# yizhiwang96/Slice3D

Measured on AMD Instinct MI355X. Metric: occupancy query-points/sec (U-Net encode + per-query decode, 256^2 x 12 slices), higher is better.
Workload: dtype f16x3

## Files before the change

### include/slice3d_hip.h

```cpp
#ifndef SLICE3D_HIP_H
#define SLICE3D_HIP_H

#include <stddef.h>
#include <stdint.h>

#ifdef __cplusplus
extern "C" {
#endif

#define S3D_VERSION 119
#define S3D_E_ARG (-1)
#define S3D_E_WORKSPACE (-2)

#define S3D_N_LEVELS 5
#define S3D_D_MODEL 128
#define S3D_N_LAYERS 3
#define S3D_FFN 2048
#define S3D_N_TOKENS_MAX 13

#define S3D_PREC_F32 0
#define S3D_PREC_F16X3 1
#define S3D_PREC_F16 2
#define S3D_PREC_BF16 3

int s3d_version(void);
// ... 325 lines not shown
```

### slice3d_amd/csrc/api.hip

```cpp
#include <dlfcn.h>
#include <stdarg.h>
#include <string.h>

#include <vector>
#include <mutex>

#include <math.h>

#include "conv.h"
#include "decode.h"
#include "train.h"
#include "ldm_ops.h"

static thread_local char g_err[512] = "";

void s3d_set_error(const char* fmt, ...) {
    va_list ap;
    va_start(ap, fmt);
    vsnprintf(g_err, sizeof(g_err), fmt, ap);
    va_end(ap);
}

extern "C" int s3d_version(void) { return S3D_VERSION; }
extern "C" const char* s3d_last_error(void) { return g_err; }
// ... 100 lines not shown
static const bool kEncTap[13] = {false, true, false, true, false, false, true,
                                 false, false, true, false, false, true};
static const int kUpC[4] = {512, 256, 128, 64};

struct PackedConv {
    size_t w, scale, shift;
    size_t w16;
    int cout_pad, KU;
};
struct EncLayout {
    PackedConv enc[13];
    size_t pool_scale[4], pool_shift[4];
};
struct UNetLayout {
    EncLayout E;
    PackedConv trans_c, trans_up[4], up_t[4], up_c1[4], up_c2[4], outc;
    size_t emds;
    size_t enc0_raw;
    size_t total;
};

static int pad16(int c) { return (c + 15) / 16 * 16; }

struct ImageAlloc {
    size_t off = 0;
    size_t take(size_t n) {
        size_t o = off;
        off += (n + 3) / 4 * 4;
        return o;
    }
    void conv(PackedConv& pc, int cout_pad, int KU) {
        pc.cout_pad = cout_pad;
        pc.KU = KU;
        pc.w = take((size_t)cout_pad * KU * 16);
        pc.w16 = take((size_t)cout_pad * KU * 16);
        pc.scale = take(cout_pad);
        pc.shift = take(cout_pad);
    }
};

static EncLayout enc_layout(ImageAlloc& a) {
    EncLayout E;
    for (int i = 0; i < 13; ++i) a.conv(E.enc[i], kEncCout[i], 9 * pad16(kEncCin[i]) / 16);
    const int tapc[4] = {64, 128, 256, 512};
    for (int i = 0; i < 4; ++i) {
        E.pool_scale[i] = a.take(tapc[i]);
        E.pool_shift[i] = a.take(tapc[i]);
    }
    return E;
}

static UNetLayout unet_layout(int n_slices) {
    UNetLayout L;
    ImageAlloc a;
    L.E = enc_layout(a);
    a.conv(L.trans_c, 512, 640 / 16);
    for (int i = 0; i < 4; ++i) {
        const int C = kUpC[i], Ct = C / 2;
        a.conv(L.trans_up[i], Ct, C / 16);
        a.conv(L.up_t[i], 4 * Ct, C / 16);
        a.conv(L.up_c1[i], Ct, 2 * 9 * Ct / 16);
        a.conv(L.up_c2[i], Ct, 9 * Ct / 16);
    }
    a.conv(L.outc, 16, 32 / 16);
    L.emds = a.take((size_t)n_slices * 128);
    L.enc0_raw = a.take(64 * 27);
    L.total = a.off;
    return L;
}

extern "C" size_t s3d_unet_packed_bytes(int n_slices) { return unet_layout(n_slices).total * sizeof(float); }

static int pack_conv3(const float* w, float* dst, int cout, int cout_pad, int cin_tot, int cin_begin, int cseg,
                      int KU_total, int u_off, int taps, hipStream_t st, int f16 = 0) {
    PackArgs a = {};
    a.f16 = f16;
// ... 22 lines not shown
        TRY(pack_conv3(P[i].w, base + pc.w, kEncCout[i], pc.cout_pad, kEncCin[i], 0, kEncCin[i], pc.KU, 0, 9, st));
        if (kEncCin[i] % 32 == 0)
            TRY(pack_conv3(P[i].w, base + pc.w16, kEncCout[i], pc.cout_pad, kEncCin[i], 0, kEncCin[i], pc.KU, 0, 9, st, 1));
        if (kEncTap[i])
            TRY(launch_fold_bn(P[i].b, nullptr, base + pc.scale, base + pc.shift, kEncCout[i], pc.cout_pad, 1, 0, st));
        else
            TRY(launch_fold_bn(P[i].b, P[i].bn, base + pc.scale, base + pc.shift, kEncCout[i], pc.cout_pad, 1, 1, st));
    }
    const int tapi[4] = {1, 3, 6, 9};
    for (int i = 0; i < 4; ++i)
        TRY(launch_fold_bn(nullptr, P[tapi[i]].bn, base + E.pool_scale[i], base + E.pool_shift[i], kEncCout[tapi[i]],
                           kEncCout[tapi[i]], 1, 0, st));
    return 0;
}

extern "C" int s3d_unet_pack(const S3dUNetParams* P, void* packed, size_t packed_bytes, void* stream) {
    hipStream_t st = (hipStream_t)stream;
    S3D_CHECK_ARG(P && packed, "unet_pack: null argument");
    S3D_CHECK_ARG(P->n_slices >= 1 && P->n_slices <= 12, "unet_pack: n_slices %d", P->n_slices);
    const UNetLayout L = unet_layout(P->n_slices);
    if (packed_bytes < L.total * sizeof(float)) {
        s3d_set_error("unet_pack: packed buffer %zu < %zu bytes", packed_bytes, L.total * sizeof(float));
        return S3D_E_WORKSPACE;
    }
    float* base = (float*)packed;
    TRY(pack_encoder(P->enc, base, L.E, st));
    if (hipMemcpyAsync(base + L.enc0_raw, P->enc[0].w, 64 * 27 * sizeof(float), hipMemcpyDeviceToDevice, st) != hipSuccess) {
        s3d_set_error("unet_pack: copy of conv1_1's weight failed");
        return S3D_E_ARG;
    }
    TRY(pack_linear(P->trans_c.w, base + L.trans_c.w, 512, 512, 640, 640, 0, st));
    TRY(pack_linear(P->trans_c.w, base + L.trans_c.w16, 512, 512, 640, 640, 0, st, 1));
    TRY(launch_fold_bn(P->trans_c.b, nullptr, base + L.trans_c.scale, base + L.trans_c.shift, 512, 512, 1, 0, st));
    for (int i = 0; i < 4; ++i) {
        const int C = kUpC[i], Ct = C / 2;
        TRY(pack_linear(P->trans_up[i].w, base + L.trans_up[i].w, Ct, Ct, C, C, 0, st));
        TRY(pack_linear(P->trans_up[i].w, base + L.trans_up[i].w16, Ct, Ct, C, C, 0, st, 1));
        TRY(launch_fold_bn(P->trans_up[i].b, nullptr, base + L.trans_up[i].scale, base + L.trans_up[i].shift, Ct,
                           Ct, 1, 0, st));
        {
            PackArgs a = {};
            a.src = P->up_t[i].w; a.dst = base + L.up_t[i].w; a.kind = S3D_PACK_CONVT;
            a.n_valid = 4 * Ct; a.n_pad = 4 * Ct; a.KU_total = C / 16; a.u_off = 0; a.ku_seg = C / 16;
            a.k_valid = C; a.ct = Ct;
            TRY(launch_pack(a, st));
            a.f16 = 1; a.dst = base + L.up_t[i].w16;
            TRY(launch_pack(a, st));
            TRY(launch_fold_bn(P->up_t[i].b, nullptr, base + L.up_t[i].scale, base + L.up_t[i].shift, Ct, 4 * Ct, 4,
                               0, st));
        }
        TRY(pack_conv3(P->up_c1[i].w, base + L.up_c1[i].w, Ct, Ct, C, 0, Ct, L.up_c1[i].KU, 0, 9, st));
        TRY(pack_conv3(P->up_c1[i].w, base + L.up_c1[i].w, Ct, Ct, C, Ct, Ct, L.up_c1[i].KU, 9 * Ct / 16, 9, st));
        TRY(pack_conv3(P->up_c1[i].w, base + L.up_c1[i].w16, Ct, Ct, C, 0, Ct, L.up_c1[i].KU, 0, 9, st, 1));
        TRY(pack_conv3(P->up_c1[i].w, base + L.up_c1[i].w16, Ct, Ct, C, Ct, Ct, L.up_c1[i].KU, 9 * Ct / 16, 9, st, 1));
        TRY(launch_fold_bn(nullptr, P->up_c1[i].bn, base + L.up_c1[i].scale, base + L.up_c1[i].shift, Ct, Ct, 1, 0,
                           st));
        TRY(pack_conv3(P->up_c2[i].w, base + L.up_c2[i].w, Ct, Ct, Ct, 0, Ct, L.up_c2[i].KU, 0, 9, st));
        TRY(pack_conv3(P->up_c2[i].w, base + L.up_c2[i].w16, Ct, Ct, Ct, 0, Ct, L.up_c2[i].KU, 0, 9, st, 1));
        TRY(launch_fold_bn(nullptr, P->up_c2[i].bn, base + L.up_c2[i].scale, base + L.up_c2[i].shift, Ct, Ct, 1, 0,
                           st));
    }
    TRY(pack_linear(P->outc.w, base + L.outc.w, 3, 16, 32, 32, 0, st));
    TRY(pack_linear(P->outc.w, base + L.outc.w16, 3, 16, 32, 32, 0, st, 1));
    TRY(launch_fold_bn(P->outc.b, nullptr, base + L.outc.scale, base + L.outc.shift, 3, 16, 1, 0, st));
    hipError_t e = hipMemcpyAsync(base + L.emds, P->emds, (size_t)P->n_slices * 128 * sizeof(float),
                                  hipMemcpyDeviceToDevice, st);
    if (e != hipSuccess) {
        s3d_set_error("unet_pack: memcpy failed: %s", hipGetErrorString(e));
        return (int)e;
    }
    return 0;
}

#define S3D_SPLITK_FLOATS ((size_t)4718592)
struct UNetWs {
    size_t in16, a, b, x[5], p[4], proj, up, mid, splitk;
    size_t total;
};
static UNetWs unet_ws(int B, int S, int ns) {
    UNetWs W;
    size_t off = 0;
    auto take = [&](size_t n) {
        size_t o = off;
        off += (n + 63) / 64 * 64;
        return o;
    };
    const size_t px = (size_t)B * S * S;
    W.in16 = take(px * 16);
    W.a = take(px * 64);
    W.b = take(px * 64 / 2);
    const int xc[5] = {64, 128, 256, 512, 512};
    for (int i = 0; i < 5; ++i) W.x[i] = take((px >> (2 * i)) * xc[i]);
    for (int i = 0; i < 4; ++i) W.p[i] = take((px >> (2 * (i + 1))) * xc[i]);
    W.proj = take(px * 32);
    W.up = take(px * ns * 32);
    W.mid = take(px * ns * 32);
    W.splitk = take(S3D_SPLITK_FLOATS);
    W.total = off;
    return W;
}

extern "C" size_t s3d_unet_workspace_bytes(int batch, int size, int n_slices) {
    return unet_ws(batch, size, n_slices).total * sizeof(float);
}

static ConvLaunch conv_desc(const float* base, const PackedConv& pc, int prec, int N, int H, int W, int ks, int act) {
    ConvLaunch c = {};
    c.wpk16 = prec != S3D_PREC_F32 ? (const void*)(base + pc.w16) : nullptr;
    c.single_pass = prec == S3D_PREC_F16;
    c.N = N; c.H = H; c.W = W; c.ks = ks;
    c.CoutPad = pc.cout_pad; c.wpk = base + pc.w; c.KU = pc.KU;
    c.scale = base + pc.scale; c.shift = base + pc.shift;
// ... 2 lines not shown
}
static ConvSrc plain_src(const float* p, int C) { return ConvSrc{p, C, 1, 0, 0}; }

static ConvLaunch proj_desc(const float* w, const void* w16, bool single, int n, int k, const float* x, int N, int H,
                            int W, float* out, const float* shift = nullptr, int act = S3D_ACT_NONE) {
    ConvLaunch c = {};
    c.N = N; c.H = H; c.W = W; c.ks = 1;
    c.CoutPad = n; c.wpk = w; c.KU = k / 16;
    c.wpk16 = w16; c.single_pass = single;
    c.shift = shift; c.act = act;
    c.out_mode = S3D_OUT_NHWC; c.cout_store = n; c.out_cstride = n;
    c.nsrc = 1;
    c.src[0] = plain_src(x, k);
    c.out = out;
    return c;
}

static int encoder_fwd(const float* base, const EncLayout& E, int prec, int N, int S, int first, const float* in,
                       float* const tap[5], float* const pp[2], float* const pool[4], float* splitk, hipStream_t st) {
    const float* cur = in;
    int curC = first ? kEncCout[0] : 16, res = S, tap_i = 0, flip = first;
    for (int i = first; i < 13; ++i) {
        ConvLaunch c = conv_desc(base, E.enc[i], prec, N, res, res, 3, kEncTap[i] ? S3D_ACT_NONE : S3D_ACT_RELU);
        c.nsrc = 1;
        c.src[0] = plain_src(cur, curC);
        c.splitk_ws = splitk; c.splitk_floats = S3D_SPLITK_FLOATS;
        c.out = kEncTap[i] ? tap[tap_i] : pp[flip];
        TRY(launch_conv(c, st));
        cur = c.out;
        curC = kEncCout[i];
// ... 29 lines not shown
        s3d_set_error("unet_encode: workspace %zu < %zu bytes", workspace_bytes, W.total * sizeof(float));
        return S3D_E_WORKSPACE;
    }
    const float* base = (const float*)packed;
    float* ws = (float*)workspace;

    ProfScope prof_(S3D_PROF_UNET, st);
    float* const pp[2] = {ws + W.a, ws + W.b};
    float* const tap[5] = {ws + W.x[0], ws + W.x[1], ws + W.x[2], ws + W.x[3], ws + W.x[4]};
    float* const pool[4] = {ws + W.p[0], ws + W.p[1], ws + W.p[2], ws + W.p[3]};
    TRY(launch_conv3x3_first(img, 3, base + L.enc0_raw, nullptr, pp[0], B, S, S, st, base + L.E.enc[0].scale,
                             base + L.E.enc[0].shift, 1));
    TRY(encoder_fwd(base, L.E, prec, B, S, 1, pp[0], tap, pp, pool, ws + W.splitk, st));
    const int r5 = S / 16;
    {
        ConvLaunch c = conv_desc(base, L.trans_c, prec, B * ns, r5, r5, 1, S3D_ACT_NONE);
        c.nsrc = 2;
        c.src[0] = ConvSrc{ws + W.x[4], 512, ns, 0, 0};
        c.src[1] = ConvSrc{base + L.emds, 128, 1, ns, 1};
        c.out = out->level[0];
        TRY(launch_conv(c, st));
    }
    const float* prev = out->level[0];
    int rp = r5;
    for (int i = 0; i < 4; ++i) {
        const int C = kUpC[i], Ct = C / 2, ro = rp * 2;
        {
            ConvLaunch c = conv_desc(base, L.trans_up[i], prec, B, ro, ro, 1, S3D_ACT_NONE);
            c.nsrc = 1;
            c.src[0] = plain_src(ws + W.x[3 - i], C);
            c.out = ws + W.proj;
            TRY(launch_conv(c, st));
        }
        {
            ConvLaunch c = conv_desc(base, L.up_t[i], prec, B * ns, rp, rp, 1, S3D_ACT_NONE);
            c.nsrc = 1;
            c.src[0] = plain_src(prev, C);
            c.out = ws + W.up;
            c.out_mode = S3D_OUT_CONVT;
            c.cout_store = Ct;
            TRY(launch_conv(c, st));
        }
        {
            ConvLaunch c = conv_desc(base, L.up_c1[i], prec, B * ns, ro, ro, 3, S3D_ACT_RELU);
            c.nsrc = 2;
            c.src[0] = ConvSrc{ws + W.proj, Ct, ns, 0, 0};
            c.src[1] = plain_src(ws + W.up, Ct);
            c.out = ws + W.mid;
            TRY(launch_conv(c, st));
        }
        {
            ConvLaunch c = conv_desc(base, L.up_c2[i], prec, B * ns, ro, ro, 3, S3D_ACT_RELU);
            c.nsrc = 1;
            c.src[0] = plain_src(ws + W.mid, Ct);
            c.out = out->level[i + 1];
            TRY(launch_conv(c, st));
        }
        prev = out->level[i + 1];
        rp = ro;
    }
    if (slices_rec) {
        ConvLaunch c = conv_desc(base, L.outc, prec, B * ns, S, S, 1, S3D_ACT_TANH);
        c.nsrc = 1;
        c.src[0] = plain_src(prev, 32);
// ... 687 lines not shown
```

### slice3d_amd/csrc/conv.h

```cpp
#pragma once
#include "common.h"
#include "dropout.h"

struct ConvSrc {
    const float* p;
    int C;
    int bdiv, bmod, sbcast;
};

#define S3D_GN_SLICES 64
#define S3D_GN_CMAX 1536
struct ConvGn {
    const float* table;
    int silu;
};

enum { S3D_ACT_NONE = 0, S3D_ACT_RELU = 1, S3D_ACT_TANH = 2 };
enum { S3D_OUT_NHWC = 0, S3D_OUT_CONVT = 1, S3D_OUT_NCHW = 2 };

struct ConvLaunch {
    ConvSrc src[2];
    int nsrc;
    int N, H, W;
    int ks;
// ... 10 lines not shown
    int act;
    float* out;
    int out_mode;
    int cout_store;
    int out_cstride;
    const float* residual;
    int out_accumulate;
    int xcd_remap;
    const float* gate;
    float gate_scale;
    unsigned long long drop_base;
    float* splitk_ws;
    size_t splitk_floats;
    DropCfg drop;
    ConvGn gn;
    int* splits_out;
};

int launch_conv(const ConvLaunch& a, hipStream_t stream);
int launch_conv_splitk_finish(const ConvLaunch& a, int nsplit, hipStream_t stream);

enum { S3D_PACK_LINEAR = 0, S3D_PACK_CONV = 1, S3D_PACK_CONVT = 2, S3D_PACK_CONV_DGRAD = 3,
       S3D_PACK_CONVT_DGRAD = 4, S3D_PACK_LINEAR_T = 5 };
struct PackArgs {
    const float* src;
    float* dst;
    int kind;
    int n_valid, n_pad;
    int KU_total, u_off, ku_seg;
    int ld, k_valid;
// ... 16 lines not shown
};
class PackBatchSuspend {
public:
    PackBatchSuspend();
    ~PackBatchSuspend();
private:
    void* saved_;
};
int launch_fold_bn(const float* bias, const float* const bn[4], float* scale, float* shift, int c_valid,
                   int c_pad, int rep, int bias_before_bn, hipStream_t stream);

int launch_bn_relu_pool(const float* in, const float* scale, const float* shift, float* out, int n, int h,
                        int w, int c, hipStream_t stream);
int launch_nchw_to_nhwc(const float* in, float* out, int n, int c, int h, int w, int cpad, hipStream_t stream);
int launch_nhwc_to_nchw(const float* in, float* out, int n, int c, int h, int w, hipStream_t stream);
int launch_add_nchw(const float* a, const float* b, float* out, int n, int c, int h, int w, hipStream_t stream);

int launch_vgg_prep(const float* pred, const float* target, const float* mean, const float* stdv, float* out,
                    int n_img, int size, hipStream_t stream);
int launch_vgg_first_f16x3(const float* pred, const float* target, const float* mean, const float* stdv, const float* w_oihw,
                           const float* bias, float* out, int n_img, int size, hipStream_t stream);
int launch_l1_diff(const float* a, const float* b, long n, float scale, float* partial, float* loss_acc,
                   hipStream_t stream);
```

### slice3d_amd/csrc/conv.hip

```cpp
#include <stdlib.h>
#include "conv.h"
#include <vector>

template <int MT, int NT>
__device__ __forceinline__ void conv_epilogue(const ConvLaunch& a, f32x4 (&acc)[MT][NT], const int (&pn)[MT],
                                              const int (&py)[MT], const int (&px)[MT], const bool (&pv)[MT],
                                              int jt0, int g) {
    const bool convt32 = a.out_mode == S3D_OUT_CONVT && a.cout_store % 32 == 0;
    if (NT % 2 == 0 && (a.out_mode == S3D_OUT_NHWC || convt32)) {
        const int m = threadIdx.x & 15;
        const bool lo = m < 8;
#pragma unroll
        for (int np = 0; np < NT / 2; ++np) {
            const int co = (jt0 + 2 * np) * 16 + 16 * (m >> 3) + 4 * g;
            const f32x4 sc = a.scale ? ld4(a.scale + co) : f32x4{1.f, 1.f, 1.f, 1.f};
            const f32x4 sh = a.shift ? ld4(a.shift + co) : zero4();
            const int ct = a.cout_store, cq = convt32 ? co / ct : 0, ccol = convt32 ? co - cq * ct : co;
            const bool col_ok = convt32 ? cq < 4 : co < a.cout_store;
#pragma unroll
            for (int mt = 0; mt < MT; ++mt) {
                f32x4 val[2];
                s3d_full_line_pair(acc[mt][2 * np], acc[mt][2 * np + 1], m, val[0], val[1]);
                const long ob = convt32 ? ((long)(pn[mt] * 2 * a.H + 2 * py[mt] + (cq >> 1)) * (2 * a.W) + 2 * px[mt] + (cq & 1)) * ct
                                        : ((long)(pn[mt] * a.H + py[mt]) * a.W + px[mt]) * a.out_cstride;
// ... 67 lines not shown
                const int ct = a.cout_store;
                const int q = co / ct, c = co - q * ct;
                if (q < 4) {
                    const int oy = 2 * py[mt] + (q >> 1), ox = 2 * px[mt] + (q & 1);
                    float* o = a.out + ((long)(pn[mt] * 2 * a.H + oy) * (2 * a.W) + ox) * ct + c;
                    st4(o, v);
                }
            } else {
#pragma unroll
                for (int i = 0; i < 4; ++i)
                    if (co + i < a.cout_store)
                        a.out[((long)(pn[mt] * a.cout_store + co + i) * a.H + py[mt]) * a.W + px[mt]] = v[i];
            }
        }
    }
}

__device__ __forceinline__ void conv_block_tile(const ConvLaunch& a, int n_co_blk, int& blk_co, long& blk_px) {
    const long L = blockIdx.x;
    if (!a.xcd_remap || n_co_blk == 1) {
        blk_co = (int)(L % n_co_blk);
        blk_px = L / n_co_blk;
        return;
    }
    const long n_px = gridDim.x / n_co_blk, full = n_px & ~7L, lim = full * n_co_blk;
    if (L < lim) {
        const long k = L >> 3;
        blk_co = (int)(k % n_co_blk);
        blk_px = (k / n_co_blk) * 8 + (L & 7);
    } else {
        const long r = L - lim;
        blk_co = (int)(r % n_co_blk);
        blk_px = full + r / n_co_blk;
    }
}

template <int MT, int NT, int WM, int WN, int KS>
__global__ __launch_bounds__(WM* WN * 64) void conv_igemm_kernel(const ConvLaunch a) {
    const int lane = threadIdx.x & 63;
    const int wave = threadIdx.x >> 6;
    const int wm = wave % WM, wn = wave / WM;
    const int m = lane & 15, g = lane >> 4;
    constexpr int PIX_WG = WM * MT * 16;
    constexpr int CO_WG = WN * NT * 16;
    const long P = (long)a.N * a.H * a.W;
    const int n_co_blk = a.CoutPad / CO_WG;
    int blk_co;
    long blk_px;
    conv_block_tile(a, n_co_blk, blk_co, blk_px);
    const int HW = a.H * a.W;
    const int stride = a.stride > 1 ? a.stride : 1;
    const int Hin = a.Hin ? a.Hin : a.H, Win = a.Win ? a.Win : a.W;
    const int PAD = a.pad_origin ? 0 : (KS == 3 ? 1 : 0);

    int pn[MT], py[MT], px[MT];
    bool pv[MT];
#pragma unroll
    for (int mt = 0; mt < MT; ++mt) {
        const long p = blk_px * PIX_WG + (long)(wm * MT + mt) * 16 + m;
        pv[mt] = p < P;
        const long pc = pv[mt] ? p : 0;
        pn[mt] = (int)(pc / HW);
        const int r = (int)(pc - (long)pn[mt] * HW);
        py[mt] = r / a.W;
        px[mt] = r - py[mt] * a.W;
    }

    f32x4 acc[MT][NT];
#pragma unroll
    for (int mt = 0; mt < MT; ++mt)
#pragma unroll
        for (int nt = 0; nt < NT; ++nt) acc[mt][nt] = zero4();

    const int jt0 = blk_co * (CO_WG / 16) + wn * NT;
    int ubase = 0;
#pragma unroll 1
    for (int s = 0; s < a.nsrc; ++s) {
        const ConvSrc S = a.src[s];
        const int cu = S.C >> 4;
#pragma unroll 1
        for (int tap = 0; tap < KS * KS; ++tap) {
            const int dy = tap / KS - PAD, dx = tap % KS - PAD;
            const float* bp[MT];
            bool ok[MT];
#pragma unroll
            for (int mt = 0; mt < MT; ++mt) {
                const int y = py[mt] * stride + dy, x = px[mt] * stride + dx;
                ok[mt] = pv[mt] && y >= 0 && y < Hin && x >= 0 && x < Win;
                const int ni = (S.bmod ? pn[mt] % S.bmod : pn[mt]) / S.bdiv;
// ... 8 lines not shown
                for (int mt = 0; mt < MT; ++mt) b[mt] = ok[mt] ? ld4(bp[mt] + 16 * c) : zero4();
#pragma unroll
                for (int nt = 0; nt < NT; ++nt) w[nt] = ld4(wp + ((size_t)nt * a.KU + c) * 256);
#pragma unroll
                for (int mt = 0; mt < MT; ++mt)
#pragma unroll
                    for (int nt = 0; nt < NT; ++nt) acc[mt][nt] += mfma4(w[nt], b[mt], zero4());
            }
        }
        ubase += KS * KS * cu;
    }

    conv_epilogue<MT, NT>(a, acc, pn, py, px, pv, jt0, g);
}

template <int MT, int NT, int WM, int WN, int KS>
__global__ __launch_bounds__(WM* WN * 64) void conv_igemm_f16x3_kernel(const ConvLaunch a) {
    const int lane = threadIdx.x & 63;
    const int wave = threadIdx.x >> 6;
    const int wm = wave % WM, wn = wave / WM;
    const int m = lane & 15, g = lane >> 4;
    constexpr int PIX_WG = WM * MT * 16;
    constexpr int CO_WG = WN * NT * 16;
    const long P = (long)a.N * a.H * a.W;
    const int n_co_blk = a.CoutPad / CO_WG;
    int blk_co;
    long blk_px;
    conv_block_tile(a, n_co_blk, blk_co, blk_px);
    const int HW = a.H * a.W;
    const int stride = a.stride > 1 ? a.stride : 1;
    const int Hin = a.Hin ? a.Hin : a.H, Win = a.Win ? a.Win : a.W;
// ... 1 lines not shown
    const int KU32 = a.KU >> 1;
    const _Float16* wimg = reinterpret_cast<const _Float16*>(a.wpk16);

    int pn[MT], py[MT], px[MT];
    bool pv[MT];
#pragma unroll
    for (int mt = 0; mt < MT; ++mt) {
        const long p = blk_px * PIX_WG + (long)(wm * MT + mt) * 16 + m;
        pv[mt] = p < P;
        const long pc = pv[mt] ? p : 0;
        pn[mt] = (int)(pc / HW);
        const int r = (int)(pc - (long)pn[mt] * HW);
        py[mt] = r / a.W;
        px[mt] = r - py[mt] * a.W;
    }
    f32x4 acc[MT][NT];
#pragma unroll
    for (int mt = 0; mt < MT; ++mt)
#pragma unroll
        for (int nt = 0; nt < NT; ++nt) acc[mt][nt] = zero4();

    const int jt0 = blk_co * (CO_WG / 16) + wn * NT;
    int ubase = 0;
#pragma unroll 1
    for (int s = 0; s < a.nsrc; ++s) {
        const ConvSrc S = a.src[s];
        const int cu = S.C >> 5;
#pragma unroll 1
        for (int tap = 0; tap < KS * KS; ++tap) {
            const int dy = tap / KS - PAD, dx = tap % KS - PAD;
            const float* bp[MT];
            bool ok[MT];
#pragma unroll
            for (int mt = 0; mt < MT; ++mt) {
                const int y = py[mt] * stride + dy, x = px[mt] * stride + dx;
                ok[mt] = pv[mt] && y >= 0 && y < Hin && x >= 0 && x < Win;
                const int ni = (S.bmod ? pn[mt] % S.bmod : pn[mt]) / S.bdiv;
// ... 413 lines not shown
__device__ unsigned long long c3_stamps[4][8];
#define C3_STAMP(i)                                                                                              \
    do {                                                                                                         \
        const long long t__ = wall_clock64();                                                                    \
        if (threadIdx.x == 0) atomicAdd(&c3_stamps[c3_cls][i], (unsigned long long)(t__ - c3_last));              \
        c3_last = t__;                                                                                           \
    } while (0)
extern "C" void s3d_debug_c3_stamps(unsigned long long* out) {
    unsigned long long z[32] = {0};
    (void)hipMemcpyFromSymbol(out, HIP_SYMBOL(c3_stamps), sizeof(z));
    (void)hipMemcpyToSymbol(HIP_SYMBOL(c3_stamps), z, sizeof(z));
}
#else
#define C3_STAMP(i)
#endif
template <int MT, int WP, int WC, int NBUF, bool GN = false>
__global__ __launch_bounds__(256) void conv3x3_lds_f16x3_kernel(const ConvLaunch a, int tiles_x, int tiles_y,
                                                                int chunks_per_split) {
    static_assert(MT * WP == 8 && WP * WC == 4, "tile is 8 rows, 4 waves");
    constexpr int NT = 2, CO_WG = WC * NT * 16;
    __shared__ __attribute__((aligned(16))) _Float16 s_in[NBUF][2][C3_HALO * C3_PXS];
    __shared__ __attribute__((aligned(16))) float s_gn[GN ? 2 * S3D_GN_CMAX : 4];
#ifdef C3_STAMPS
    long long c3_last = wall_clock64();
    const int c3_cls = gridDim.x == 96 ? 0 : gridDim.x == 48 ? 1 : gridDim.x == 12 ? 2 : 3;
    if (threadIdx.x == 0) atomicAdd(&c3_stamps[c3_cls][7], 1ull);
#endif
    const int lane = threadIdx.x & 63, wave = threadIdx.x >> 6;
    const int m = lane & 15, g = lane >> 4;
    const int wp = wave % WP, wc = wave / WP;
    const int n_co_blk = a.CoutPad / CO_WG;
    int blk_co;
// ... 70 lines not shown
    const int ch_lo = blockIdx.y * chunks_per_split;
    const int nchunk = min(cu0 + cu1, ch_lo + chunks_per_split);
    fetch(a.src[ch_lo < cu0 ? 0 : 1], ch_lo < cu0 ? ch_lo : ch_lo - cu0, ch_lo < cu0 ? 0 : a.src[0].C);
    if (GN) {
        const int Ct = a.src[0].C + (a.nsrc > 1 ? a.src[1].C : 0);
        const float* tb = a.gn.table + (size_t)n * 2 * Ct;
        for (int i = threadIdx.x; i < Ct / 4; i += 256) {
            st4(s_gn + 4 * i, ld4(tb + 4 * i));
            st4(s_gn + S3D_GN_CMAX + 4 * i, ld4(tb + Ct + 4 * i));
        }
        __syncthreads();
    }
    C3_STAMP(0);
    park(ch_lo & (NBUF - 1));
    C3_STAMP(1);
    __syncthreads();
    C3_STAMP(2);
#pragma unroll 1
    for (int ch = ch_lo; ch < nchunk; ++ch) {
        const int s = ch < cu0 ? 0 : 1, c = s ? ch - cu0 : ch, cu = s ? cu1 : cu0;
        const int ubase = s ? 9 * cu0 : 0;
        const _Float16* wp0 = wimg + ((size_t)jt0 * KU32 + ubase + c) * 1024 + lane * 8;
        s3d_half8 wh[NT], wl[NT];
#pragma unroll
        for (int nt = 0; nt < NT; ++nt) {
            const _Float16* f = wp0 + (size_t)nt * KU32 * 1024;
            wh[nt] = *reinterpret_cast<const s3d_half8*>(f);
            wl[nt] = *reinterpret_cast<const s3d_half8*>(f + 512);
        }
        if (ch + 1 < nchunk) {
// ... 364 lines not shown
            return 0;
        }
        return launch_conv_splitk_finish(a, splits, stream);
    }
    dim3 grid((unsigned)nblk, (unsigned)splits);
    constexpr int one_buf_max = 2;
    const bool one = cps <= one_buf_max;
    if (a.gn.table) {
        int ct = 0;
        for (int s = 0; s < a.nsrc; ++s) ct += a.src[s].C;
        S3D_CHECK_ARG(ct <= S3D_GN_CMAX, "conv: fused GroupNorm over %d channels", ct);
        if (co_wg == 64)
            hipLaunchKernelGGL((conv3x3_lds_f16x3_kernel<4, 2, 2, 2, true>), grid, dim3(256), 0, stream, a, tiles_x, tiles_y, cps);
        else
            hipLaunchKernelGGL((conv3x3_lds_f16x3_kernel<2, 4, 1, 2, true>), grid, dim3(256), 0, stream, a, tiles_x, tiles_y, cps);
    } else if (co_wg == 64) {
        hipLaunchKernelGGL((conv3x3_lds_f16x3_kernel<4, 2, 2, 2>), grid, dim3(256), 0, stream, a, tiles_x, tiles_y, cps);
    } else {
        if (one) hipLaunchKernelGGL((conv3x3_lds_f16x3_kernel<2, 4, 1, 1>), grid, dim3(256), 0, stream, a, tiles_x, tiles_y, cps);
        else hipLaunchKernelGGL((conv3x3_lds_f16x3_kernel<2, 4, 1, 2>), grid, dim3(256), 0, stream, a, tiles_x, tiles_y, cps);
    }
    S3D_LAUNCH_CHECK();
    if (a.splits_out) {
        *a.splits_out = splits;
        if (splits > 1) return 0;
    }
    if (splits > 1) return launch_conv_splitk_finish(a, splits, stream);
    return 0;
}

template <int MT, int NT, int WM, int WN>
static int launch_cfg(const ConvLaunch& a, hipStream_t stream) {
    constexpr int PIX_WG = WM * MT * 16, CO_WG = WN * NT * 16;
    const long P = (long)a.N * a.H * a.W;
    const long nblk = ((P + PIX_WG - 1) / PIX_WG) * (a.CoutPad / CO_WG);
    S3D_CHECK_ARG(nblk > 0 && nblk < (1L << 31), "conv grid out of range (%ld)", nblk);
    dim3 grid((unsigned)nblk), block(WM * WN * 64);
    bool f16 = a.wpk16 != nullptr && (a.KU % 2 == 0);
    for (int s = 0; s < a.nsrc; ++s) f16 = f16 && (a.src[s].C % 32 == 0);
    if (f16) {
        if (a.ks == 3)
            hipLaunchKernelGGL((conv_igemm_f16x3_kernel<MT, NT, WM, WN, 3>), grid, block, 0, stream, a);
        else if (a.ks == 2)
            hipLaunchKernelGGL((conv_igemm_f16x3_kernel<MT, NT, WM, WN, 2>), grid, block, 0, stream, a);
        else
            hipLaunchKernelGGL((conv_igemm_f16x3_kernel<MT, NT, WM, WN, 1>), grid, block, 0, stream, a);
        S3D_LAUNCH_CHECK();
        return 0;
    }
    if (a.ks == 3)
        hipLaunchKernelGGL((conv_igemm_kernel<MT, NT, WM, WN, 3>), grid, block, 0, stream, a);
    else if (a.ks == 2)
        hipLaunchKernelGGL((conv_igemm_kernel<MT, NT, WM, WN, 2>), grid, block, 0, stream, a);
    else
// ... 1 lines not shown
    S3D_LAUNCH_CHECK();
    return 0;
}

int launch_conv(const ConvLaunch& a_in, hipStream_t stream) {
    ConvLaunch a = a_in;
    a.xcd_remap = 1;
    S3D_CHECK_ARG(a.ks >= 1 && a.ks <= 3, "conv: ks must be 1, 2 or 3");
    S3D_CHECK_ARG(!a.pad_origin || (a.ks == 3 && a.stride > 1 && a.out_mode == S3D_OUT_NHWC),
                  "conv: pad_origin is served for strided 3x3 convolutions only");
    S3D_CHECK_ARG(a.CoutPad % 16 == 0 && a.CoutPad > 0, "conv: CoutPad %d", a.CoutPad);
    for (int s = 0; s < a.nsrc; ++s)
        S3D_CHECK_ARG(a.src[s].C % 16 == 0 && a.src[s].bdiv >= 1, "conv: bad source %d", s);
    S3D_CHECK_ARG(a.out_mode != S3D_OUT_CONVT || (a.drop.p <= 0.f && !a.gate && !a.residual && !a.out_accumulate),
                  "conv: ConvTranspose output takes no dropout / gate / residual / accumulate");
    if (conv3x3_lds_eligible(a)) return launch_conv3x3_lds(a, stream);
    S3D_CHECK_ARG(!a.gn.table, "conv: a fused GroupNorm needs the LDS-staged 3x3 kernel (ks 3, stride 1, channel counts multiples of 32)");
    if (conv1x1_small_eligible(a)) {
        bool served = false;
        const int rc = launch_conv1x1_small(a, stream, served);
        if (rc || served) return rc;
    }
    if (lin_stream_eligible(a)) return launch_lin_stream(a, stream);
    if (lin_rows_eligible(a)) return launch_lin_rows(a, stream);
    const long P = (long)a.N * a.H * a.W;
    const long want = 512;
    auto nblk = [&](int pix, int co) { return ((P + pix - 1) / pix) * (a.CoutPad / co); };
    if (a.CoutPad % 128 == 0) {
        if (nblk(128, 128) >= want) return launch_cfg<4, 4, 2, 2>(a, stream);
        if (nblk(64, 128) >= want) return launch_cfg<2, 4, 2, 2>(a, stream);
// ... 218 lines not shown
        r /= h;
        const int cc = (int)(r % c);
        const int ni = (int)(r / c);
        out[idx] = in[((long)(ni * h + y) * w + x) * c + cc];
    }
}

int launch_nchw_to_nhwc(const float* in, float* out, int n, int c, int h, int w, int cpad, hipStream_t stream) {
    const long total = (long)n * h * w * cpad;
    const int blocks = (int)((total + 255) / 256 < 8192 ? (total + 255) / 256 : 8192);
    hipLaunchKernelGGL(nchw_to_nhwc_kernel, dim3(blocks), dim3(256), 0, stream, in, out, n, c, h, w, cpad);
    S3D_LAUNCH_CHECK();
    return 0;
}

__global__ void add_nchw_kernel(const float* __restrict__ a, const float* __restrict__ b, float* __restrict__ out, int n, int c,
                                int h, int w) {
    const long total = (long)n * h * w * c;
    for (long idx = (long)blockIdx.x * blockDim.x + threadIdx.x; idx < total; idx += (long)gridDim.x * blockDim.x) {
        const int cc = (int)(idx % c);
        long r = idx / c;
        const int x = (int)(r % w);
        r /= w;
        const int y = (int)(r % h);
        const int ni = (int)(r / h);
        out[idx] = a[idx] + b[((long)(ni * c + cc) * h + y) * w + x];
    }
}
int launch_add_nchw(const float* a, const float* b, float* out, int n, int c, int h, int w, hipStream_t stream) {
    const long total = (long)n * h * w * c;
// ... 168 lines not shown
```

Measured before the change: 11.65 million.

## Factor slice-embedding terms out of U-Net bottleneck and first up-block convolutions

Splits the trans_c 1x1 conv into an image term computed once per batch and a per-slice embedding term precomputed at pack time, combined by a broadcast-add kernel. The skip-connection half of each up_c1 conv is now computed once per batch image and injected as an accumulator initial value (a new PRE path in the conv kernels), instead of being recomputed for every slice. For the first up block, the linear chain through the ConvTranspose and 3x3 conv is applied to the shared latent once, and the slice-dependent part becomes a small per-slice border/parity table added in an activation kernel. This removes redundant per-slice convolution work, at the cost of extra workspace, new kernel variants and more launches.

```diff
diff --git a/include/slice3d_hip.h b/include/slice3d_hip.h
--- a/include/slice3d_hip.h
+++ b/include/slice3d_hip.h
@@ -8,7 +8,7 @@
 extern "C" {
 #endif
 
-#define S3D_VERSION 119
+#define S3D_VERSION 120
 #define S3D_E_ARG (-1)
 #define S3D_E_WORKSPACE (-2)
 
diff --git a/slice3d_amd/csrc/api.hip b/slice3d_amd/csrc/api.hip
--- a/slice3d_amd/csrc/api.hip
+++ b/slice3d_amd/csrc/api.hip
@@ -138,7 +138,12 @@
 };
 struct UNetLayout {
     EncLayout E;
-    PackedConv trans_c, trans_up[4], up_t[4], up_c1[4], up_c2[4], outc;
+    PackedConv trans_up[4], up_t[4], up_c1[4], up_c2[4], outc;
+    PackedConv trans_cx, trans_ce;
+    size_t slice_v;
+    size_t up1_tab;
+    size_t up1_tab_in;
+    PackedConv up_c1s[4];
     size_t emds;
     size_t enc0_raw;
     size_t total;
@@ -161,6 +166,13 @@
         pc.scale = take(cout_pad);
         pc.shift = take(cout_pad);
     }
+    void weights(PackedConv& pc, int cout_pad, int KU) {
+        pc.cout_pad = cout_pad;
+        pc.KU = KU;
+        pc.w = take((size_t)cout_pad * KU * 16);
+        pc.w16 = take((size_t)cout_pad * KU * 16);
+        pc.scale = pc.shift = 0;
+    }
 };
 
 static EncLayout enc_layout(ImageAlloc& a) {
@@ -178,12 +190,17 @@
     UNetLayout L;
     ImageAlloc a;
     L.E = enc_layout(a);
-    a.conv(L.trans_c, 512, 640 / 16);
+    a.conv(L.trans_cx, 512, 512 / 16);
+    a.weights(L.trans_ce, 512, 128 / 16);
+    L.slice_v = a.take((size_t)n_slices * 512);
+    L.up1_tab = a.take((size_t)n_slices * 16 * 256);
+    L.up1_tab_in = a.take((size_t)n_slices * 16 * 256);
     for (int i = 0; i < 4; ++i) {
         const int C = kUpC[i], Ct = C / 2;
         a.conv(L.trans_up[i], Ct, C / 16);
         a.conv(L.up_t[i], 4 * Ct, C / 16);
-        a.conv(L.up_c1[i], Ct, 2 * 9 * Ct / 16);
+        a.weights(L.up_c1s[i], Ct, 9 * Ct / 16);
+        a.conv(L.up_c1[i], Ct, 9 * Ct / 16);
         a.conv(L.up_c2[i], Ct, 9 * Ct / 16);
     }
     a.conv(L.outc, 16, 32 / 16);
@@ -236,6 +253,8 @@
     return 0;
 }
 
+static int pack_unet_slice_terms(float* base, const UNetLayout& L, int ns, hipStream_t st);
+
 extern "C" int s3d_unet_pack(const S3dUNetParams* P, void* packed, size_t packed_bytes, void* stream) {
     hipStream_t st = (hipStream_t)stream;
     S3D_CHECK_ARG(P && packed, "unet_pack: null argument");
@@ -251,9 +270,10 @@
         s3d_set_error("unet_pack: copy of conv1_1's weight failed");
         return S3D_E_ARG;
     }
-    TRY(pack_linear(P->trans_c.w, base + L.trans_c.w, 512, 512, 640, 640, 0, st));
-    TRY(pack_linear(P->trans_c.w, base + L.trans_c.w16, 512, 512, 640, 640, 0, st, 1));
-    TRY(launch_fold_bn(P->trans_c.b, nullptr, base + L.trans_c.scale, base + L.trans_c.shift, 512, 512, 1, 0, st));
+    TRY(pack_linear(P->trans_c.w, base + L.trans_cx.w, 512, 512, 512, 640, 0, st));
+    TRY(pack_linear(P->trans_c.w, base + L.trans_cx.w16, 512, 512, 512, 640, 0, st, 1));
+    TRY(launch_fold_bn(P->trans_c.b, nullptr, base + L.trans_cx.scale, base + L.trans_cx.shift, 512, 512, 1, 0, st));
+    TRY(pack_linear(P->trans_c.w + 512, base + L.trans_ce.w, 512, 512, 128, 640, 0, st));
     for (int i = 0; i < 4; ++i) {
         const int C = kUpC[i], Ct = C / 2;
         TRY(pack_linear(P->trans_up[i].w, base + L.trans_up[i].w, Ct, Ct, C, C, 0, st));
@@ -271,10 +291,10 @@
             TRY(launch_fold_bn(P->up_t[i].b, nullptr, base + L.up_t[i].scale, base + L.up_t[i].shift, Ct, 4 * Ct, 4,
                                0, st));
         }
-        TRY(pack_conv3(P->up_c1[i].w, base + L.up_c1[i].w, Ct, Ct, C, 0, Ct, L.up_c1[i].KU, 0, 9, st));
-        TRY(pack_conv3(P->up_c1[i].w, base + L.up_c1[i].w, Ct, Ct, C, Ct, Ct, L.up_c1[i].KU, 9 * Ct / 16, 9, st));
-        TRY(pack_conv3(P->up_c1[i].w, base + L.up_c1[i].w16, Ct, Ct, C, 0, Ct, L.up_c1[i].KU, 0, 9, st, 1));
-        TRY(pack_conv3(P->up_c1[i].w, base + L.up_c1[i].w16, Ct, Ct, C, Ct, Ct, L.up_c1[i].KU, 9 * Ct / 16, 9, st, 1));
+        TRY(pack_conv3(P->up_c1[i].w, base + L.up_c1s[i].w, Ct, Ct, C, 0, Ct, L.up_c1s[i].KU, 0, 9, st));
+        TRY(pack_conv3(P->up_c1[i].w, base + L.up_c1[i].w, Ct, Ct, C, Ct, Ct, L.up_c1[i].KU, 0, 9, st));
+        TRY(pack_conv3(P->up_c1[i].w, base + L.up_c1s[i].w16, Ct, Ct, C, 0, Ct, L.up_c1s[i].KU, 0, 9, st, 1));
+        TRY(pack_conv3(P->up_c1[i].w, base + L.up_c1[i].w16, Ct, Ct, C, Ct, Ct, L.up_c1[i].KU, 0, 9, st, 1));
         TRY(launch_fold_bn(nullptr, P->up_c1[i].bn, base + L.up_c1[i].scale, base + L.up_c1[i].shift, Ct, Ct, 1, 0,
                            st));
         TRY(pack_conv3(P->up_c2[i].w, base + L.up_c2[i].w, Ct, Ct, Ct, 0, Ct, L.up_c2[i].KU, 0, 9, st));
@@ -291,12 +311,13 @@
         s3d_set_error("unet_pack: memcpy failed: %s", hipGetErrorString(e));
         return (int)e;
     }
-    return 0;
+    return pack_unet_slice_terms(base, L, P->n_slices, st);
 }
 
 #define S3D_SPLITK_FLOATS ((size_t)4718592)
 struct UNetWs {
-    size_t in16, a, b, x[5], p[4], proj, up, mid, splitk;
+    size_t in16, a, b, x[5], p[4], proj, pre, up, mid, splitk;
+    size_t lat, up1_u, up1_pre;
     size_t total;
 };
 static UNetWs unet_ws(int B, int S, int ns) {
@@ -315,9 +336,13 @@
     for (int i = 0; i < 5; ++i) W.x[i] = take((px >> (2 * i)) * xc[i]);
     for (int i = 0; i < 4; ++i) W.p[i] = take((px >> (2 * (i + 1))) * xc[i]);
     W.proj = take(px * 32);
+    W.pre = take(px * 32);
     W.up = take(px * ns * 32);
     W.mid = take(px * ns * 32);
     W.splitk = take(S3D_SPLITK_FLOATS);
+    W.lat = take(px / 256 * 512);
+    W.up1_u = take(px / 64 * 256);
+    W.up1_pre = take(px / 64 * 256);
     W.total = off;
     return W;
 }
@@ -350,6 +375,35 @@
     c.src[0] = plain_src(x, k);
     c.out = out;
     return c;
+}
+
+static int pack_unet_slice_terms(float* base, const UNetLayout& L, int ns, hipStream_t st) {
+    {
+        ConvLaunch c = conv_desc(base, L.trans_ce, S3D_PREC_F32, ns, 1, 1, 1, S3D_ACT_NONE);
+        c.scale = nullptr; c.shift = base + L.trans_cx.shift;
+        c.nsrc = 1;
+        c.src[0] = plain_src(base + L.emds, 128);
+        c.out = base + L.slice_v;
+        TRY(launch_conv(c, st));
+    }
+    {
+        ConvLaunch c = conv_desc(base, L.up_t[0], S3D_PREC_F32, ns, 2, 2, 1, S3D_ACT_NONE);
+        c.nsrc = 1;
+        c.src[0] = ConvSrc{base + L.slice_v, 512, 1, 0, 1};
+        c.out = base + L.up1_tab_in;
+        c.out_mode = S3D_OUT_CONVT;
+        c.cout_store = 256;
+        TRY(launch_conv(c, st));
+    }
+    {
+        ConvLaunch c = conv_desc(base, L.up_c1[0], S3D_PREC_F32, ns, 4, 4, 3, S3D_ACT_NONE);
+        c.scale = c.shift = nullptr;
+        c.nsrc = 1;
+        c.src[0] = plain_src(base + L.up1_tab_in, 256);
+        c.out = base + L.up1_tab;
+        TRY(launch_conv(c, st));
+    }
+    return 0;
 }
 
 static int encoder_fwd(const float* base, const EncLayout& E, int prec, int N, int S, int first, const float* in,
@@ -409,13 +463,14 @@
     TRY(encoder_fwd(base, L.E, prec, B, S, 1, pp[0], tap, pp, pool, ws + W.splitk, st));
     const int r5 = S / 16;
     {
-        ConvLaunch c = conv_desc(base, L.trans_c, prec, B * ns, r5, r5, 1, S3D_ACT_NONE);
-        c.nsrc = 2;
-        c.src[0] = ConvSrc{ws + W.x[4], 512, ns, 0, 0};
-        c.src[1] = ConvSrc{base + L.emds, 128, 1, ns, 1};
-        c.out = out->level[0];
+        ConvLaunch c = conv_desc(base, L.trans_cx, prec, B, r5, r5, 1, S3D_ACT_NONE);
+        c.scale = c.shift = nullptr;
+        c.nsrc = 1;
+        c.src[0] = plain_src(ws + W.x[4], 512);
+        c.out = ws + W.lat;
         TRY(launch_conv(c, st));
     }
+    TRY(launch_slice_bcast_add(ws + W.lat, base + L.slice_v, out->level[0], B, ns, (long)r5 * r5, 512, st));
     const float* prev = out->level[0];
     int rp = r5;
     for (int i = 0; i < 4; ++i) {
@@ -428,21 +483,53 @@
             TRY(launch_conv(c, st));
         }
         {
-            ConvLaunch c = conv_desc(base, L.up_t[i], prec, B * ns, rp, rp, 1, S3D_ACT_NONE);
+            ConvLaunch c = conv_desc(base, L.up_c1s[i], prec, B, ro, ro, 3, S3D_ACT_NONE);
+            c.scale = c.shift = nullptr;
             c.nsrc = 1;
-            c.src[0] = plain_src(prev, C);
-            c.out = ws + W.up;
-            c.out_mode = S3D_OUT_CONVT;
-            c.cout_store = Ct;
+            c.src[0] = plain_src(ws + W.proj, Ct);
+            c.out = ws + W.pre;
             TRY(launch_conv(c, st));
         }
-        {
-            ConvLaunch c = conv_desc(base, L.up_c1[i], prec, B * ns, ro, ro, 3, S3D_ACT_RELU);
-            c.nsrc = 2;
-            c.src[0] = ConvSrc{ws + W.proj, Ct, ns, 0, 0};
-            c.src[1] = plain_src(ws + W.up, Ct);
-            c.out = ws + W.mid;
-            TRY(launch_conv(c, st));
+        if (i == 0) {
+            {
+                ConvLaunch c = conv_desc(base, L.up_t[0], prec, B, rp, rp, 1, S3D_ACT_NONE);
+                c.scale = c.shift = nullptr;
+                c.nsrc = 1;
+                c.src[0] = plain_src(ws + W.lat, C);
+                c.out = ws + W.up1_u;
+                c.out_mode = S3D_OUT_CONVT;
+                c.cout_store = Ct;
+                TRY(launch_conv(c, st));
+            }
+            {
+                ConvLaunch c = conv_desc(base, L.up_c1[0], prec, B, ro, ro, 3, S3D_ACT_NONE);
+                c.scale = c.shift = nullptr;
+                c.nsrc = 1;
+                c.src[0] = plain_src(ws + W.up1_u, Ct);
+                c.pre = ws + W.pre; c.pre_bdiv = 1;
+                c.out = ws + W.up1_pre;
+                TRY(launch_conv(c, st));
+            }
+            TRY(launch_slice_table_act(ws + W.up1_pre, base + L.up1_tab, base + L.up_c1[0].scale, base + L.up_c1[0].shift,
+                                       ws + W.mid, B, ns, ro, Ct, st));
+        } else {
+            {
+                ConvLaunch c = conv_desc(base, L.up_t[i], prec, B * ns, rp, rp, 1, S3D_ACT_NONE);
+                c.nsrc = 1;
+                c.src[0] = plain_src(prev, C);
+                c.out = ws + W.up;
+                c.out_mode = S3D_OUT_CONVT;
+                c.cout_store = Ct;
+                TRY(launch_conv(c, st));
+            }
+            {
+                ConvLaunch c = conv_desc(base, L.up_c1[i], prec, B * ns, ro, ro, 3, S3D_ACT_RELU);
+                c.nsrc = 1;
+                c.src[0] = plain_src(ws + W.up, Ct);
+                c.pre = ws + W.pre; c.pre_bdiv = ns;
+                c.out = ws + W.mid;
+                TRY(launch_conv(c, st));
+            }
         }
         {
             ConvLaunch c = conv_desc(base, L.up_c2[i], prec, B * ns, ro, ro, 3, S3D_ACT_RELU);
diff --git a/slice3d_amd/csrc/conv.h b/slice3d_amd/csrc/conv.h
--- a/slice3d_amd/csrc/conv.h
+++ b/slice3d_amd/csrc/conv.h
@@ -48,6 +48,8 @@
     size_t splitk_floats;
     DropCfg drop;
     ConvGn gn;
+    const float* pre;
+    int pre_bdiv, pre_bmod;
     int* splits_out;
 };
 
@@ -94,6 +96,9 @@
                         int w, int c, hipStream_t stream);
 int launch_nchw_to_nhwc(const float* in, float* out, int n, int c, int h, int w, int cpad, hipStream_t stream);
 int launch_nhwc_to_nchw(const float* in, float* out, int n, int c, int h, int w, hipStream_t stream);
+int launch_slice_bcast_add(const float* a, const float* v, float* out, int B, int ns, long npix, int C, hipStream_t stream);
+int launch_slice_table_act(const float* a, const float* tab, const float* scale, const float* shift, float* out, int B, int ns,
+                           int R, int C, hipStream_t stream);
 int launch_add_nchw(const float* a, const float* b, float* out, int n, int c, int h, int w, hipStream_t stream);
 
 int launch_vgg_prep(const float* pred, const float* target, const float* mean, const float* stdv, float* out,
diff --git a/slice3d_amd/csrc/conv.hip b/slice3d_amd/csrc/conv.hip
--- a/slice3d_amd/csrc/conv.hip
+++ b/slice3d_amd/csrc/conv.hip
@@ -105,6 +105,13 @@
             }
         }
     }
+}
+
+template <bool PRE>
+__device__ __forceinline__ f32x4 conv_acc_init(const ConvLaunch& a, bool valid, int n, int y, int x, int co) {
+    if (!PRE || !valid) return zero4();
+    const int ni = (a.pre_bmod ? n % a.pre_bmod : n) / a.pre_bdiv;
+    return ld4(a.pre + ((long)(ni * a.H + y) * a.W + x) * a.CoutPad + co);
 }
 
 __device__ __forceinline__ void conv_block_tile(const ConvLaunch& a, int n_co_blk, int& blk_co, long& blk_px) {
@@ -126,7 +133,7 @@
     }
 }
 
-template <int MT, int NT, int WM, int WN, int KS>
+template <int MT, int NT, int WM, int WN, int KS, bool PRE = false>
 __global__ __launch_bounds__(WM* WN * 64) void conv_igemm_kernel(const ConvLaunch a) {
     const int lane = threadIdx.x & 63;
     const int wave = threadIdx.x >> 6;
@@ -157,13 +164,13 @@
         px[mt] = r - py[mt] * a.W;
     }
 
+    const int jt0 = blk_co * (CO_WG / 16) + wn * NT;
     f32x4 acc[MT][NT];
 #pragma unroll
     for (int mt = 0; mt < MT; ++mt)
 #pragma unroll
-        for (int nt = 0; nt < NT; ++nt) acc[mt][nt] = zero4();
-
-    const int jt0 = blk_co * (CO_WG / 16) + wn * NT;
+        for (int nt = 0; nt < NT; ++nt) acc[mt][nt] = conv_acc_init<PRE>(a, pv[mt], pn[mt], py[mt], px[mt], (jt0 + nt) * 16 + 4 * g);
+
     int ubase = 0;
 #pragma unroll 1
     for (int s = 0; s < a.nsrc; ++s) {
@@ -202,7 +209,7 @@
     conv_epilogue<MT, NT>(a, acc, pn, py, px, pv, jt0, g);
 }
 
-template <int MT, int NT, int WM, int WN, int KS>
+template <int MT, int NT, int WM, int WN, int KS, bool PRE = false>
 __global__ __launch_bounds__(WM* WN * 64) void conv_igemm_f16x3_kernel(const ConvLaunch a) {
     const int lane = threadIdx.x & 63;
     const int wave = threadIdx.x >> 6;
@@ -234,13 +241,13 @@
         py[mt] = r / a.W;
         px[mt] = r - py[mt] * a.W;
     }
+    const int jt0 = blk_co * (CO_WG / 16) + wn * NT;
     f32x4 acc[MT][NT];
 #pragma unroll
     for (int mt = 0; mt < MT; ++mt)
 #pragma unroll
-        for (int nt = 0; nt < NT; ++nt) acc[mt][nt] = zero4();
-
-    const int jt0 = blk_co * (CO_WG / 16) + wn * NT;
+        for (int nt = 0; nt < NT; ++nt) acc[mt][nt] = conv_acc_init<PRE>(a, pv[mt], pn[mt], py[mt], px[mt], (jt0 + nt) * 16 + 4 * g);
+
     int ubase = 0;
 #pragma unroll 1
     for (int s = 0; s < a.nsrc; ++s) {
@@ -684,8 +691,8 @@
 #else
 #define C3_STAMP(i)
 #endif
-template <int MT, int WP, int WC, int NBUF, bool GN = false>
-__global__ __launch_bounds__(256) void conv3x3_lds_f16x3_kernel(const ConvLaunch a, int tiles_x, int tiles_y,
+template <int MT, int WP, int WC, int NBUF, bool GN = false, bool PRE = false>
+__global__ __launch_bounds__(256, (PRE && MT == 2) ? 3 : 1) void conv3x3_lds_f16x3_kernel(const ConvLaunch a, int tiles_x, int tiles_y,
                                                                 int chunks_per_split) {
     static_assert(MT * WP == 8 && WP * WC == 4, "tile is 8 rows, 4 waves");
     constexpr int NT = 2, CO_WG = WC * NT * 16;
@@ -786,6 +793,14 @@
     C3_STAMP(0);
     park(ch_lo & (NBUF - 1));
     C3_STAMP(1);
+    if (PRE) {
+#pragma unroll
+        for (int mt = 0; mt < MT; ++mt) {
+            const int y = y0 + MT * wp + mt, x = x0 + m;
+#pragma unroll
+            for (int nt = 0; nt < NT; ++nt) acc[mt][nt] = conv_acc_init<true>(a, y < a.H && x < a.W, n, y, x, (jt0 + nt) * 16 + 4 * g);
+        }
+    }
     __syncthreads();
     C3_STAMP(2);
 #pragma unroll 1
@@ -1180,6 +1195,11 @@
             hipLaunchKernelGGL((conv3x3_lds_f16x3_kernel<4, 2, 2, 2, true>), grid, dim3(256), 0, stream, a, tiles_x, tiles_y, cps);
         else
             hipLaunchKernelGGL((conv3x3_lds_f16x3_kernel<2, 4, 1, 2, true>), grid, dim3(256), 0, stream, a, tiles_x, tiles_y, cps);
+    } else if (a.pre) {
+        if (co_wg == 64)
+            hipLaunchKernelGGL((conv3x3_lds_f16x3_kernel<4, 2, 2, 2, false, true>), grid, dim3(256), 0, stream, a, tiles_x, tiles_y, cps);
+        else
+            hipLaunchKernelGGL((conv3x3_lds_f16x3_kernel<2, 4, 1, 2, false, true>), grid, dim3(256), 0, stream, a, tiles_x, tiles_y, cps);
     } else if (co_wg == 64) {
         hipLaunchKernelGGL((conv3x3_lds_f16x3_kernel<4, 2, 2, 2>), grid, dim3(256), 0, stream, a, tiles_x, tiles_y, cps);
     } else {
@@ -1204,6 +1224,12 @@
     dim3 grid((unsigned)nblk), block(WM * WN * 64);
     bool f16 = a.wpk16 != nullptr && (a.KU % 2 == 0);
     for (int s = 0; s < a.nsrc; ++s) f16 = f16 && (a.src[s].C % 32 == 0);
+    if (a.pre) {
+        if (f16) hipLaunchKernelGGL((conv_igemm_f16x3_kernel<MT, NT, WM, WN, 3, true>), grid, block, 0, stream, a);
+        else hipLaunchKernelGGL((conv_igemm_kernel<MT, NT, WM, WN, 3, true>), grid, block, 0, stream, a);
+        S3D_LAUNCH_CHECK();
+        return 0;
+    }
     if (f16) {
         if (a.ks == 3)
             hipLaunchKernelGGL((conv_igemm_f16x3_kernel<MT, NT, WM, WN, 3>), grid, block, 0, stream, a);
@@ -1235,6 +1261,11 @@
         S3D_CHECK_ARG(a.src[s].C % 16 == 0 && a.src[s].bdiv >= 1, "conv: bad source %d", s);
     S3D_CHECK_ARG(a.out_mode != S3D_OUT_CONVT || (a.drop.p <= 0.f && !a.gate && !a.residual && !a.out_accumulate),
                   "conv: ConvTranspose output takes no dropout / gate / residual / accumulate");
+    S3D_CHECK_ARG(!a.pre || (a.ks == 3 && a.stride <= 1 && !a.Hin && !a.Win), "conv: a pre-activation addend is served for 3x3 stride-1 convolutions only");
+    S3D_CHECK_ARG(!a.pre || a.out_mode != S3D_OUT_CONVT, "conv: a pre-activation addend with a ConvTranspose output");
+    S3D_CHECK_ARG(!a.pre || !a.splitk_ws, "conv: a pre-activation addend with a split-K workspace");
+    S3D_CHECK_ARG(!a.pre || !a.gn.table, "conv: a pre-activation addend with a fused GroupNorm");
+    S3D_CHECK_ARG(!a.pre || (a.pre_bdiv >= 1 && a.pre_bmod >= 0), "conv: addend image rule bdiv %d bmod %d", a.pre_bdiv, a.pre_bmod);
     if (conv3x3_lds_eligible(a)) return launch_conv3x3_lds(a, stream);
     S3D_CHECK_ARG(!a.gn.table, "conv: a fused GroupNorm needs the LDS-staged 3x3 kernel (ks 3, stride 1, channel counts multiples of 32)");
     if (conv1x1_small_eligible(a)) {
@@ -1483,6 +1514,58 @@
     return 0;
 }
 
+__global__ __launch_bounds__(256) void slice_bcast_add_kernel(const float* __restrict__ a, const float* __restrict__ v,
+                                                              float* __restrict__ out, int ns, long npix, int C, long total) {
+    const int cq = C >> 2;
+    for (long idx = (long)blockIdx.x * blockDim.x + threadIdx.x; idx < total; idx += (long)gridDim.x * blockDim.x) {
+        const int c = (int)(idx % cq) * 4;
+        const long ip = idx / cq, img = ip / npix, p = ip - img * npix;
+        const long b = img / ns;
+        const int s = (int)(img - b * ns);
+        const f32x4 r = ld4(a + (b * npix + p) * C + c) + ld4(v + (long)s * C + c);
+        __builtin_nontemporal_store(r, reinterpret_cast<f32x4*>(out + idx * 4));
+    }
+}
+int launch_slice_bcast_add(const float* a, const float* v, float* out, int B, int ns, long npix, int C, hipStream_t stream) {
+    S3D_CHECK_ARG(a && v && out && B >= 1 && ns >= 1 && npix >= 1 && C >= 4 && C % 4 == 0, "slice_bcast_add: bad argument");
+    const long total = (long)B * ns * npix * (C >> 2);
+    const int blocks = (int)((total + 255) / 256 < 4096 ? (total + 255) / 256 : 4096);
+    hipLaunchKernelGGL(slice_bcast_add_kernel, dim3(blocks), dim3(256), 0, stream, a, v, out, ns, npix, C, total);
+    S3D_LAUNCH_CHECK();
+    return 0;
+}
+
+__global__ __launch_bounds__(256) void slice_table_act_kernel(const float* __restrict__ a, const float* __restrict__ tab,
+                                                              const float* __restrict__ scale, const float* __restrict__ shift,
+                                                              float* __restrict__ out, int ns, int R, int C, long total) {
+    const int cq = C >> 2;
+    for (long idx = (long)blockIdx.x * blockDim.x + threadIdx.x; idx < total; idx += (long)gridDim.x * blockDim.x) {
+        const int c = (int)(idx % cq) * 4;
+        long ip = idx / cq;
+        const int x = (int)(ip % R);
+        ip /= R;
+        const int y = (int)(ip % R);
+        const long img = ip / R, b = img / ns;
+        const int s = (int)(img - b * ns);
+        const int cy = y == 0 ? 0 : y == R - 1 ? 3 : (y & 1) ? 1 : 2, cx = x == 0 ? 0 : x == R - 1 ? 3 : (x & 1) ? 1 : 2;
+        f32x4 r = ld4(a + ((b * R + y) * R + x) * C + c) + ld4(tab + (long)((s * 4 + cy) * 4 + cx) * C + c);
+        r = r * ld4(scale + c) + ld4(shift + c);
+#pragma unroll
+        for (int i = 0; i < 4; ++i) r[i] = fmaxf(r[i], 0.f);
+        __builtin_nontemporal_store(r, reinterpret_cast<f32x4*>(out + idx * 4));
+    }
+}
+int launch_slice_table_act(const float* a, const float* tab, const float* scale, const float* shift, float* out, int B, int ns,
+                           int R, int C, hipStream_t stream) {
+    S3D_CHECK_ARG(a && tab && scale && shift && out && B >= 1 && ns >= 1 && R >= 2 && C >= 4 && C % 4 == 0,
+                  "slice_table_act: bad argument");
+    const long total = (long)B * ns * R * R * (C >> 2);
+    const int blocks = (int)((total + 255) / 256 < 4096 ? (total + 255) / 256 : 4096);
+    hipLaunchKernelGGL(slice_table_act_kernel, dim3(blocks), dim3(256), 0, stream, a, tab, scale, shift, out, ns, R, C, total);
+    S3D_LAUNCH_CHECK();
+    return 0;
+}
+
 __global__ void add_nchw_kernel(const float* __restrict__ a, const float* __restrict__ b, float* __restrict__ out, int n, int c,
                                 int h, int w) {
     const long total = (long)n * h * w * c;
```

After: 11.77 million, median of 6. +1.1%, better.
